# hydradarpa/kalman-hydra

Hardware: AMD Instinct MI355X
Metric: frames/sec (Brox flow + EKF update) at 1024^2 (higher is better)
Workload: dtype f32 (flow, renders) / f64 (EKF sums and state)

## Files before the change

kalman-hydra_amd/csrc/dense_kernels.h:

```cpp
#pragma once
#include <hip/hip_runtime.h>
#include "ekf_kernels.h"
#include "host_block.h"

#define DNB 32
#define TTT_PF 3

__device__ __forceinline__ double d_rsqrt(double d)
{
    const double r = __builtin_amdgcn_rsq(d);
    const double e = fma(-(d * r), r, 1.0);
#ifdef HM_RSQRT_ORDER2
    return fma(r * 0.5, e, r);
#else
    return fma(r, fma(e, 0.375, 0.5) * e, r);
#endif
}

__device__ __forceinline__ double d_readlane(double v, int lane)
{
    const int lo = __builtin_amdgcn_readlane(__double2loint(v), lane);
    const int hi = __builtin_amdgcn_readlane(__double2hiint(v), lane);
    return __hiloint2double(hi, lo);
}
// ... 438 lines not shown
    const int jj = 16 * (wv & 1) + (lane & 15);
#pragma unroll
    for (int e = 0; e < 4; e++) {
        const int ii = 16 * (wv >> 1) + (lane >> 4) + 4 * e;
        if (ii < ni && jj < nj) {
            W[(size_t)(i0 + ii) * n + j0 + jj] = acc[e];
            W[(size_t)(j0 + jj) * n + i0 + ii] = acc[e];
        }
    }
}

__global__ __launch_bounds__(256) void k_assemble(const double *__restrict__ invW0, const double *__restrict__ H,
                                                  const double *__restrict__ X0, const double *__restrict__ X,
                                                  const double *__restrict__ Hz, double *__restrict__ A, int n, int rhs_row,
                                                  double *__restrict__ Lt)
{
    __shared__ double s[4];
    const int row = blockIdx.x;
    if (row == (int)gridDim.x - 1) {
        __shared__ double W[DNB][DNB + 1];
        const int nd = min(DNB, n);
        for (int e = threadIdx.x; e < DNB * DNB; e += 256) {
            const int i = e / DNB, j = e % DNB;
            W[i][j] = (i < nd && j < nd) ? invW0[(size_t)i * n + j] + H[(size_t)i * n + j] : (i == j ? 1.0 : 0.0);
        }
        __syncthreads();
        if (threadIdx.x < 64) chol32_tinv_wave(W, Lt, threadIdx.x);
        return;
    }
    if (row >= n) {
        if (row != rhs_row)
            for (int j = threadIdx.x; j < n; j += 256) A[(size_t)row * n + j] = 0.0;
        return;
    }
    double acc = 0.0;
    for (int j = threadIdx.x; j < n; j += 256) {
        const double h = H[(size_t)row * n + j];
        A[(size_t)row * n + j] = invW0[(size_t)row * n + j] + h;
        acc += h * (X0[j] + -1.0 * X[j]);
    }
    for (int o = 32; o > 0; o >>= 1) acc += __shfl_down(acc, o, 64);
    if ((threadIdx.x & 63) == 0) s[threadIdx.x >> 6] = acc;
    __syncthreads();
    if (threadIdx.x == 0) A[(size_t)rhs_row * n + row] = Hz[row] - (((s[0] + s[1]) + s[2]) + s[3]);
}

#define RES_HEAD 10

__global__ __launch_bounds__(256) void k_iter_result(const double *__restrict__ step, int n, const double *__restrict__ partial,
                                                     int ntiles, const int *__restrict__ overflow,
                                                     const unsigned *__restrict__ flow_ctl, double *__restrict__ res, double ticket,
                                                     int delay_us)
{
    __shared__ double sp[RI_GROUPS * RI_NV];
    __shared__ double sums[RI_NV];
    const int t = threadIdx.x;
    const unsigned long long stamp = hb_stamp((long long)ticket);
    d_tile_partial_sums(partial, ntiles, sp, sums);
    __syncthreads();
    double v = 0.0;
    int slot = -1;
    if (t < 4) { slot = t; v = sums[t]; }
    else if (t == 4) { slot = 4; v = (double)*overflow; }
    else if (t == 5) { slot = 5; v = ticket; }
    else if (t == 6) { slot = 6; v = 0.0; }
    else if (t == 7) { slot = 7; v = (double)flow_ctl[1]; }
    else if (t == 8) { slot = 8; v = sums[4]; }
    else if (t == 9) { slot = 9; v = sums[5]; }
    if (delay_us > 0) {
        if (t == 9) { hb_put(res, n + 9, v, stamp); hb_flush(); }
        hb_delay(delay_us);
    }
    for (int i = t; i < n; i += 256) hb_put(res, i, step[i], stamp);
    if (slot >= 0) hb_put(res, n + slot, v, stamp);
    hb_flush();
}

__global__ __launch_bounds__(256) void k_gains(const double *__restrict__ W, const double *__restrict__ Hzc, int n,
                                               double *__restrict__ out)
{
    __shared__ double sm[3][4];
    const int row = blockIdx.x;
    double a0 = 0.0, a1 = 0.0, a2 = 0.0;
    for (int j = threadIdx.x; j < n; j += 256) {
        const double w = W[(size_t)row * n + j];
        const double *c = Hzc + (size_t)4 * j;
        a0 += w * c[0];
        a1 += w * (c[1] + c[2]);
        a2 += w * c[3];
    }
    for (int o = 32; o > 0; o >>= 1) {
        a0 += __shfl_down(a0, o, 64);
        a1 += __shfl_down(a1, o, 64);
        a2 += __shfl_down(a2, o, 64);
    }
    if ((threadIdx.x & 63) == 0) {
        sm[0][threadIdx.x >> 6] = a0;
        sm[1][threadIdx.x >> 6] = a1;
        sm[2][threadIdx.x >> 6] = a2;
    }
    __syncthreads();
    if (threadIdx.x < 3) {
        const double *q = sm[threadIdx.x];
        out[(size_t)threadIdx.x * n + row] = ((q[0] + q[1]) + q[2]) + q[3];
    }
}

__global__ __launch_bounds__(1024) void k_tail_result(const double *__restrict__ Hzc, const double *__restrict__ gain, int n,
                                                      double *__restrict__ blk, double ticket, int delay_us)
{
    const unsigned long long stamp = hb_stamp((long long)ticket);
    if (delay_us > 0) {
        if (threadIdx.x == 0) { hb_put(blk, 7 * n - 1, gain[3 * n - 1], stamp); hb_flush(); }
        hb_delay(delay_us);
    }
    for (int i = threadIdx.x; i < 4 * n; i += 1024) hb_put(blk, i, Hzc[i], stamp);
    for (int i = threadIdx.x; i < 3 * n; i += 1024) hb_put(blk, 4 * n + i, gain[i], stamp);
    hb_flush();
}

struct SpringTopo {
    const int *off;
    const int *bar;
    const int *other;
    const double *blk;
};

__global__ void k_fw_rows(const double *__restrict__ W, double *__restrict__ P, int N, SpringTopo tp, double a, double s)
// ... 47 lines not shown
```

kalman-hydra_amd/csrc/ekf.hip:

```cpp
#include "hm_common.h"
#include "ekf_kernels.h"
#include "dense_kernels.h"
#include "chol_flow_kernels.h"
#include "project_kernels.h"
#include "predict_kernels.h"
#include "view_kernels.h"
#include "body_kernels.h"
#include "smooth_kernels.h"
#include <algorithm>
#include <atomic>
#include <chrono>
#include <cmath>
#include <condition_variable>
#include <cstring>
#include <functional>
#include <mutex>
#include <set>
#include <thread>
#include <utility>
#include <vector>

struct Helper {
    std::thread th;
    std::mutex m;
// ... 52 lines not shown
    HmOwner own{1};
    Helper helper;
    bool helper_used = false;
    int tail_async = 1;
    double eps_Z, eps_J, eps_M;
    hipStream_t stream;
    int *d_tri, *d_star_off, *d_star_tri, *d_edges;
    int *d_nb_off = nullptr, *d_nb_u = nullptr, *d_nb_e = nullptr;
    float *d_uv;
    uint8_t *d_tex;
    std::vector<int> edges;
    uint8_t *d_yim, *d_ym;
    float *d_yfx, *d_yfy, *d_yfxm, *d_yfym;
    bool obs_owned = true;
    const uint8_t *o_yim, *o_ym;
    const float *o_yfx, *o_yfy;
    bool have_tex, have_obs, have_ref;
    Targets ref, P, Q;
    TriSetup *d_setup, *d_cfgs;
    int4 *d_ubox;
    int *d_tlist = nullptr, *d_tcount = nullptr;
    unsigned *d_tmask = nullptr;
    double *d_X, *d_out, *d_partial;
    uint8_t *d_im8, *d_m8;
    std::vector<double> X0;
    double *d_HTH;
    double *d_H, *d_Hz, *d_Hzc, *d_invW0, *d_Af[2], *d_T[2], *d_step, *d_Wtmp, *d_X0, *d_Xn, *d_Wprior, *d_gain, *d_Awork, *d_Lt[2];
    std::vector<double> upd_X0;
    int upd_last = -1, upd_prev = -1;
    double *d_Wres;
    double *pin;
    size_t pin_n;
    int *pin_scratch;
    std::vector<double> resv, tailv;
    int result_delay = 0;
    bool tail_pending = false;
    bool tail_valid = false;
    long long tail_ticket = 0;
    hipStream_t tail_stream = nullptr;
    const uint8_t *armed_mask = nullptr;
    std::vector<int> sp_h_off, sp_h_bar, sp_h_other;
    std::vector<double> sp_h_blk;
    std::vector<int32_t> sp_bars_cached;
    std::vector<int> tri;
    DPool pool;
    int *d_area;
    int *d_sp_off, *d_sp_bar, *d_sp_other;
    double *d_sp_blk;
    bool upd_open;
    bool prefactored;
    std::vector<double> h_partial;
    int red_blocks = 512;
    double *d_tpart = nullptr;
    std::vector<double> h_tpart;
    int ntiles = 0;
    int render_rows = RI_H;
    bool last_err_valid = false;
    double last_err[4] = {0, 0, 0, 0};
    std::vector<double> last_err_X;
    long long run_ticket;
    int vsplit = 5, esplit;
    bool pn_armed = false;
    void *pn_worker = nullptr;
    std::vector<int32_t> pn_bars;
    std::vector<double> pn_l0;
    double pn_par[4] = {0, 0, 0, 0};
    int pn_maxiter = 0;
    bool pq_armed = false;
    double pq_eps_F = 0.0;
    bool pq_valid = false;
    std::vector<double> pq_X, pq_l0;
    std::vector<int32_t> pq_bars;
    double pq_par[4] = {0, 0, 0, 0};
    hipStream_t stream3 = nullptr;
    int *d_n4nbr = nullptr, *d_n4nbb = nullptr, *d_n4bars = nullptr;
    double *d_n4l0 = nullptr;
    int n4deg = 0;
    std::vector<int32_t> n4_bars;
    std::vector<double> n4_l0;
    double *pin_n4 = nullptr;
    double *d_n4X = nullptr;
    std::vector<double> n4v;
    long long n4_ticket = 0;
    bool n4_pending = false;
    int newton_fail = 0;
    hipEvent_t ev_n4 = nullptr, ev_pm = nullptr;
    bool n4_ready = false;
    bool chain_pending = false;
    std::vector<double> chain_pred, chain_proj;
    int chain_its = 0, chain_moved = 0;
    double *pin_blk = nullptr;
    std::thread worker;
    bool worker_active;
    int worker_rc;
    char worker_err[512];
    int chol_flow = 1, flow_wgs = 192;
    int flow_stall = 0;
    int speculate = 1;
    double *d_flowP;
    unsigned *d_flowctl;
    hipStream_t stream2;
    hipStream_t stream4 = nullptr;
    hipEvent_t ev_tail = nullptr;
    bool tail_on_stream4 = false;
    int tail_split = 1;
    int *d_nbars, *d_nvoff, *d_nvbar, *d_ninfo;
// ... 243 lines not shown
            if (rc == HM_OK && 4 * ((int)nb[v].size() + 1) > PREP_MAX_ENTRIES) {
                hm_set_error("hm_ctx_create: vertex %d has %d neighbours, limit %d", v, (int)nb[v].size(), PREP_MAX_ENTRIES / 4 - 1);
                rc = HM_ERR_ARG;
            }
        }
        step(upload(h->own, &h->d_nb_off, noff.data(), noff.size()));
        step(upload(h->own, &h->d_nb_u, nu.data(), nu.size()));
        step(upload(h->own, &h->d_nb_e, ne.data(), ne.size()));
    }
    hipError_t e = hipSuccess;
    auto dev = [&](auto **p, size_t bytes) { if (e == hipSuccess) e = h->own.alloc(p, bytes); };
    if (rc == HM_OK) {
        const char *pe = getenv("HYDRA_MI_EKF_PRIORITY");
        e = h->own.stream(&h->stream, !(pe && atoi(pe) == 0));
        dev(&h->d_tex, n);
        dev(&h->d_yim, n);
        dev(&h->d_ym, n);
        dev(&h->d_yfx, n * sizeof(float));
        dev(&h->d_yfy, n * sizeof(float));
        dev(&h->d_yfxm, n * sizeof(float));
        dev(&h->d_yfym, n * sizeof(float));
        dev(&h->d_setup, (size_t)T * sizeof(TriSetup));
        dev(&h->d_cfgs, (size_t)N * MEAS_NCFG * (EKF_MAX_STAR + 1) * sizeof(TriSetup));
        dev(&h->d_ubox, (size_t)N * UBOX_STRIDE * sizeof(int4));
        dev(&h->d_tmask, (size_t)N * TMASK_STRIDE * sizeof(unsigned));
        dev(&h->d_tlist, (size_t)N * TMASK_STRIDE * sizeof(int));
        dev(&h->d_tcount, (size_t)N * sizeof(int));
        dev(&h->d_X, (size_t)4 * N * sizeof(double));
        dev(&h->d_out, (size_t)h->njobs * MEAS_VSPLIT_MAX * MEAS_OUT * sizeof(double));
        dev(&h->d_partial, (size_t)h->red_blocks * 4 * sizeof(double));
        h->ntiles = hm_cdiv(W, RI_W) * hm_cdiv(H, 8);
        dev(&h->d_tpart, (size_t)h->ntiles * RI_NV * sizeof(double));
        dev(&h->d_im8, n);
        dev(&h->d_m8, n);
        const size_t n4 = (size_t)4 * N, nn = n4 * n4 * sizeof(double);
        dev(&h->d_H, nn);
        dev(&h->d_HTH, nn);
        if (e == hipSuccess) e = hipMemsetAsync(h->d_HTH, 0, nn, h->stream);
        dev(&h->d_invW0, nn);
        const size_t nn_aug = (size_t)(hm_cdiv((int)n4, DNB) * DNB + DNB) * n4 * sizeof(double);
        dev(&h->d_Af[0], nn_aug);
        dev(&h->d_Af[1], nn_aug);
        dev(&h->d_Awork, nn_aug);
        const size_t ld_bytes = (size_t)hm_cdiv((int)n4, DNB) * DNB * DNB * sizeof(double);
        dev(&h->d_T[0], nn);
        dev(&h->d_T[1], nn);
        dev(&h->d_step, n4 * sizeof(double));
        dev(&h->d_Lt[0], ld_bytes);
        dev(&h->d_Lt[1], ld_bytes);
        dev(&h->d_Wtmp, nn);
        dev(&h->d_flowP, 3 * ld_bytes);
        dev(&h->d_flowctl, 4 * sizeof(unsigned));
        if (e == hipSuccess) e = hipMemsetAsync(h->d_flowctl, 0, 4 * sizeof(unsigned), h->stream);
        dev(&h->d_Hz, n4 * sizeof(double));
        dev(&h->d_Hzc, n4 * 4 * sizeof(double));
        dev(&h->d_Wprior, nn);
        dev(&h->d_gain, n4 * 3 * sizeof(double));
        h->pin_n = 2 * (n4 + RES_HEAD + n4 * 4 + n4 * 3) + 2;
        if (e == hipSuccess) e = h->own.host_alloc(&h->pin, h->pin_n * sizeof(double), hipHostMallocCoherent);
        if (e == hipSuccess) memset(h->pin, 0, h->pin_n * sizeof(double));
        h->pin_scratch = (int *)(h->pin + h->pin_n - 2);
        h->resv.assign(n4 + RES_HEAD, 0.0);
        h->tailv.assign(n4 * 7, 0.0);
        dev(&h->d_X0, n4 * sizeof(double));
        dev(&h->pool.hdr, (size_t)4 * N * sizeof(int));
        dev(&h->pool.overflow, sizeof(int));
        dev(&h->d_area, (size_t)N * sizeof(int));
        h->pool.area = h->d_area;
        if (e == hipSuccess) e = pool_alloc(h, (long long)8 * W * H);
        dev(&h->d_Xn, n4 * sizeof(double));
        for (Targets *t : {&h->ref, &h->P, &h->Q})
            if (e == hipSuccess) e = alloc_targets(h->own, *t, n);
    }
    if (e != hipSuccess) {
        hm_set_error("hm_ctx_create: device allocation failed: %s", hipGetErrorString(e));
        step(HM_ERR_HIP);
    }
    if (rc != HM_OK) {
        ctx_free(h);
        return rc;
    }
    h->h_partial.resize((size_t)h->red_blocks * 4);
    h->h_tpart.resize((size_t)h->ntiles * RI_NV);
    *out = h;
    return HM_OK;
}

extern "C" int hm_ctx_destroy(hm_ctx_t h) { return ctx_free(h); }

#ifdef HM_STAMP
extern "C" int hm_debug_stamps(void *dev_ptr)
{
    long long *p = (long long *)dev_ptr;
    HM_HIP(hipMemcpyToSymbol(HIP_SYMBOL(g_stamp), &p, sizeof p));
    return HM_OK;
}
#endif

extern "C" int hm_ctx_tune(hm_ctx_t h, const char *key, int value)
{
    HM_ARG(h != nullptr && key != nullptr, "hm_ctx_tune: NULL argument");
    HM_JOIN(h);
    if (!strcmp(key, "measure_split")) {
        HM_ARG(value >= 1 && value <= MEAS_VSPLIT_MAX, "hm_ctx_tune: measure_split must be in 1..%d", MEAS_VSPLIT_MAX);
        h->vsplit = value;
    } else if (!strcmp(key, "chol_flow")) {
        HM_ARG(value == 0 || value == 1, "hm_ctx_tune: chol_flow must be 0 (one launch per block step) or 1 (one persistent launch)");
        h->chol_flow = value;
    } else if (!strcmp(key, "chol_flow_wgs")) {
        HM_ARG(value >= 2 && value <= 2048, "hm_ctx_tune: chol_flow_wgs must be in 2..2048 (the chain workgroup and at least one task workgroup)");
        h->flow_wgs = value;
    } else if (!strcmp(key, "render_rows")) {
        HM_ARG(value == 8 || value == 16, "hm_ctx_tune: render_rows must be 8 or 16");
        h->render_rows = value;
    } else if (!strcmp(key, "chol_flow_stall")) {
        HM_ARG(value >= 0 && value <= 100000, "hm_ctx_tune: chol_flow_stall must be in 0..100000");
        h->flow_stall = value;
    } else if (!strcmp(key, "result_delay")) {
        HM_ARG(value >= 0 && value <= 5000, "hm_ctx_tune: result_delay must be in 0..5000 (microseconds)");
        h->result_delay = value;
    } else if (!strcmp(key, "tail_async")) {
        HM_ARG(value == 0 || value == 1, "hm_ctx_tune: tail_async must be 0 or 1");
        h->tail_async = value;
    } else if (!strcmp(key, "tail_split")) {
        HM_ARG(value == 0 || value == 1, "hm_ctx_tune: tail_split must be 0 or 1");
        h->tail_split = value;
    } else if (!strcmp(key, "newton_fail")) {
        HM_ARG(value == 0 || value == 1, "hm_ctx_tune: newton_fail must be 0 or 1");
        h->newton_fail = value;
    } else if (!strcmp(key, "speculate")) {
        HM_ARG(value == 0 || value == 1, "hm_ctx_tune: speculate must be 0 or 1");
        h->speculate = value;
    } else if (!strcmp(key, "edge_split")) {
        HM_ARG(value >= 1 && value <= MEAS_VSPLIT_MAX, "hm_ctx_tune: edge_split must be in 1..%d", MEAS_VSPLIT_MAX);
        h->esplit = value;
    } else {
        hm_set_error("hm_ctx_tune: unknown key '%s'", key);
        return HM_ERR_ARG;
    }
    return HM_OK;
}
extern "C" void *hm_ctx_stream(hm_ctx_t h)
{
    (void)ctx_join(h);
    return h ? (void *)h->stream : nullptr;
}
extern "C" int hm_ctx_sync(hm_ctx_t h)
{
    HM_ARG(h != nullptr, "hm_ctx_sync: NULL handle");
    HM_JOIN(h);
    HM_HIP(hipSetDevice(h->device));
    HM_HIP(hipStreamSynchronize(h->stream));
    return HM_OK;
}

extern "C" int hm_set_texture(hm_ctx_t h, const uint8_t *tex)
{
    HM_ARG(h && tex, "hm_set_texture: NULL argument");
    HM_JOIN(h);
    HM_HIP(hipSetDevice(h->device));
    HM_HIP(hipMemcpyAsync(h->d_tex, tex, (size_t)h->W * h->H, hipMemcpyHostToDevice, h->stream));
    HM_HIP(hipStreamSynchronize(h->stream));
    h->last_err_valid = false;
    h->have_tex = true;
    return HM_OK;
}

static int ensure_stream2(hm_ctx *h)
{
    HM_HIP(h->own.stream(&h->stream2));
    return HM_OK;
}

static int project_buffers(hm_ctx *h)
{
    if (h->pm_ready) return HM_OK;
    const size_t n = (size_t)h->W * h->H, n4 = (size_t)4 * h->N;
    HM_HIP(h->own.alloc(&h->d_outline, n * sizeof(int2)));
    HM_HIP(h->own.alloc(&h->d_outline_cnt, 4 * sizeof(int)));
    HM_HIP(h->own.alloc(&h->d_pm_flag, n));
    HM_HIP(h->own.alloc(&h->d_pm_pruned, n));
    HM_HIP(h->own.alloc(&h->ccl.L, n * sizeof(int)));
    HM_HIP(h->own.alloc(&h->ccl.cnt, n * sizeof(int)));
    HM_HIP(h->own.alloc(&h->ccl.bnd, n * sizeof(int)));
    HM_HIP(h->own.alloc(&h->ccl.edge, n));
// ... 55 lines not shown
    h->o_yim = h->d_yim; h->o_ym = h->d_ym; h->o_yfx = h->d_yfx; h->o_yfy = h->d_yfy;
    int rc = finish_observation(h);
    if (rc) return rc;
    HM_HIP(hipStreamSynchronize(h->stream));
    h->outline_ready = false;
    if (h->d_outline) {
        rc = queue_outline(h, h->o_ym);
        if (rc) return rc;
        h->outline_ready = true;
    }
    return HM_OK;
}

extern "C" int hm_set_observation_dev(hm_ctx_t h, const uint8_t *d_y_im, const float *d_y_fx, const float *d_y_fy,
                                      const uint8_t *d_y_m)
{
    HM_ARG(h && d_y_im && d_y_fx && d_y_fy && d_y_m, "hm_set_observation_dev: NULL argument");
    HM_JOIN_LAZY(h);
    HM_HIP(hipSetDevice(h->device));
    h->o_yim = d_y_im; h->o_ym = d_y_m; h->o_yfx = d_y_fx; h->o_yfy = d_y_fy;
    int rc = finish_observation(h);
    if (rc) return rc;
    h->outline_ready = false;
    if (h->d_outline && h->prepared_mask == d_y_m) {
        h->outline_ready = true;
    } else if (h->d_outline) {
        rc = queue_outline(h, h->o_ym);
        if (rc) return rc;
        h->outline_ready = true;
    }
    h->prepared_mask = nullptr;
    return HM_OK;
}

static int render_dev(hm_ctx *h, const double *dX, Targets t)
{
    Mesh m = {h->W, h->H, h->N, h->T, h->d_tri, h->d_uv, h->d_tex};
    hipLaunchKernelGGL(k_setup_all, dim3(hm_cdiv(h->T, 64)), dim3(64), 0, h->stream, m, dX, h->d_setup);
    hipLaunchKernelGGL((k_render<0>), dim3(hm_cdiv(h->W, EKF_TILE), hm_cdiv(h->H, EKF_TILE)), dim3(EKF_TILE, EKF_TILE), 0,
                       h->stream, m, dX, h->d_setup, t, (const int *)nullptr, (int *)nullptr);
    HM_HIP(hipGetLastError());
    return HM_OK;
}

static int render_into(hm_ctx *h, const double *X, Targets t)
{
    HM_HIP(hipMemcpyAsync(h->d_X, X, (size_t)4 * h->N * sizeof(double), hipMemcpyHostToDevice, h->stream));
    return render_dev(h, h->d_X, t);
}

static void measure_args(hm_ctx *h, const double *dX, double deltaX, int masked, MeasureArgs &a);
static int render_strips(const hm_ctx *h) { return hm_cdiv(h->W, RI_W) * hm_cdiv(h->H, h->render_rows); }

static int render_iter(hm_ctx *h, const double *dX, Targets t, bool with_err, int masked, bool regions, double deltaX)
{
    IterRenderArgs r;
    r.m = Mesh{h->W, h->H, h->N, h->T, h->d_tri, h->d_uv, h->d_tex};
    r.X = dX;
    r.out = t;
    r.o = Obs{h->o_yim, masked ? h->d_yfxm : h->o_yfx, masked ? h->d_yfym : h->o_yfy, h->o_ym};
    r.raw_fx = h->o_yfx; r.raw_fy = h->o_yfy;
    r.partial = h->d_tpart;
    r.tiles_x = hm_cdiv(h->W, RI_W); r.tiles_y = hm_cdiv(h->H, h->render_rows);
    const int nstrips = r.tiles_x * r.tiles_y;
    r.with_err = with_err ? 1 : 0;
    r.n_regions = regions ? h->N : 0;
    MeasureArgs a;
    measure_args(h, dX, deltaX, masked, a);
    if (h->render_rows == 8) hipLaunchKernelGGL((k_render_iter<8>), dim3(r.n_regions + nstrips), dim3(256), 0, h->stream, r, a, h->d_area);
    else hipLaunchKernelGGL((k_render_iter<16>), dim3(r.n_regions + nstrips), dim3(256), 0, h->stream, r, a, h->d_area);
    HM_HIP(hipGetLastError());
    return HM_OK;
}

static void hm_tile_partial_sums(const double *p, int ntiles, double s[RI_NV])
{
    static thread_local double g[RI_GROUPS][RI_NV];
    for (int t = 0; t < RI_GROUPS; t++) {
        double a[RI_NV];
        for (int k = 0; k < RI_NV; k++) a[k] = 0.0;
        for (int i = t; i < ntiles; i += RI_GROUPS)
            for (int k = 0; k < RI_NV; k++) a[k] += p[RI_NV * (size_t)i + k];
        for (int k = 0; k < RI_NV; k++) g[t][k] = a[k];
    }
    for (int k = 0; k < RI_NV; k++) {
        double v = 0.0;
        for (int t = 0; t < RI_GROUPS; t++) v += g[t][k];
        s[k] = v;
    }
}

#define NEED_TEX(h, who) \
    if (!(h)->have_tex) { hm_set_error(who ": hm_set_texture has not been called"); return HM_ERR_STATE; }
#define NEED_OBS(h, who) \
    if (!(h)->have_obs) { hm_set_error(who ": hm_set_observation has not been called"); return HM_ERR_STATE; }
#define NEED_REF(h, who) \
    if (!(h)->have_ref) { hm_set_error(who ": hm_initjacobian has not been called"); return HM_ERR_STATE; }

extern "C" int hm_render(hm_ctx_t h, const double *X, uint8_t *im, float *fx, float *fy, uint8_t *mk)
{
    HM_ARG(h && X, "hm_render: NULL argument");
    HM_JOIN(h);
    NEED_TEX(h, "hm_render");
    HM_HIP(hipSetDevice(h->device));
    int rc = render_into(h, X, h->P);
    if (rc) return rc;
    const int n = h->W * h->H;
    hipLaunchKernelGGL(k_resolve, dim3(hm_cdiv(n, 256)), dim3(256), 0, h->stream, h->P, h->d_im8, h->d_m8, n);
    if (im) HM_HIP(hipMemcpyAsync(im, h->d_im8, n, hipMemcpyDeviceToHost, h->stream));
    if (mk) HM_HIP(hipMemcpyAsync(mk, h->d_m8, n, hipMemcpyDeviceToHost, h->stream));
    if (fx) HM_HIP(hipMemcpyAsync(fx, h->P.fx, (size_t)n * sizeof(float), hipMemcpyDeviceToHost, h->stream));
    if (fy) HM_HIP(hipMemcpyAsync(fy, h->P.fy, (size_t)n * sizeof(float), hipMemcpyDeviceToHost, h->stream));
    HM_HIP(hipStreamSynchronize(h->stream));
    return HM_OK;
}

static Obs obs_of(hm_ctx *h, int masked)
{
    Obs o = {h->o_yim, masked ? h->d_yfxm : h->o_yfx, masked ? h->d_yfym : h->o_yfy, h->o_ym};
// ... 671 lines not shown
    const auto dbg_a = std::chrono::steady_clock::now();
    auto dbg_ms = [&]() { return std::chrono::duration<double, std::milli>(std::chrono::steady_clock::now() - dbg_a).count(); };
    double dbg_stage[8] = {0, 0, 0, 0, 0, 0, 0, 0};
    int rc = update_begin(h, W_prior, chained ? nullptr : X);
    if (rc) return rc;
    dbg_stage[0] = dbg_ms();
    const int N = h->N, n4 = 4 * N;
    std::vector<double> X0, Xcur, Xold;
    if (!chained) { X0.assign(X, X + n4); Xcur = X0; Xold = X0; }
    auto chain_collect = [&]() -> int {
        int r = hb_wait(h->stream3, h->pin_n4 + n4, 0, (size_t)n4 + 2, hb_stamp(h->n4_ticket), h->n4v.data(), "hm_update_run (state prediction)");
        h->n4_pending = false;
        if (r) return r;
        r = hb_wait(h->stream3, h->pin_pm + n4, 0, (size_t)n4 + 1, hb_stamp(h->pm_ticket), h->pmv.data(), "hm_update_run (projectmask)");
        if (r) return r;
        h->chain_pred.assign(h->n4v.begin(), h->n4v.begin() + n4);
        h->chain_proj.assign(h->pmv.begin(), h->pmv.begin() + n4);
        h->chain_its = (int)h->n4v[n4];
        h->chain_moved = (int)h->pmv[n4];
        if (h->n4v[n4 + 1] != 0.0) return 2;
        X0 = h->chain_proj; Xcur = X0; Xold = X0;
        h->upd_X0 = X0;
        h->X0 = X0;
        return HM_OK;
    };
    bool collected = !chained;
    if (!chained) HM_HIP(hipMemcpyAsync(h->d_X, h->d_X0, (size_t)n4 * sizeof(double), hipMemcpyDeviceToDevice, h->stream));
    double *const pin_res = h->pin, *const pin_tail = h->pin + 2 * ((size_t)n4 + RES_HEAD);
    const double *const res = h->resv.data();
    int niter = 0, accepted = 0;
    bool reverted = false, conv = false, ref_ready = false, regions_ahead = false, grown = false;
    double eold = 0.0;
    bool spec = false;
    auto unspec = [&]() {
        if (spec) { std::swap(h->ref, h->P); std::swap(h->d_X, h->d_Xn); spec = false; }
    };
    for (int it = 0; it < max_iter; it++) {
        if (!spec) {
            rc = measure_dev(h, h->d_X, ref_ready, deltaX, masked, regions_ahead, false);
            if (rc) return rc;
        }
        spec = false;
        if (next_mask && it == 0) {
            HM_HIP(h->own.event(&h->ev_m0));
            HM_HIP(hipEventRecord(h->ev_m0, h->stream));
        }
        if (collected) h->X0 = Xcur;
        h->have_ref = true;
        const int slot = h->upd_last == 0 ? 1 : 0;
        rc = ctx_join(h);
        if (rc) return rc;
        double *rhs_row = solve_step(h, slot, deltaX);
        regions_ahead = it + 1 < max_iter;
        rc = render_iter(h, h->d_Xn, h->P, true, masked, regions_ahead, deltaX);
        if (rc) return rc;
        hipLaunchKernelGGL(k_iter_result, dim3(1), dim3(256), 0, h->stream, rhs_row, n4, h->d_tpart,
                           render_strips(h), h->pool.overflow, (const unsigned *)h->d_flowctl, pin_res, (double)(++h->run_ticket),
                           h->result_delay);
        HM_HIP(hipGetLastError());
        if (h->speculate && regions_ahead) {
            std::swap(h->ref, h->P);
            std::swap(h->d_X, h->d_Xn);
            spec = true;
            rc = measure_dev(h, h->d_X, true, deltaX, masked, true, false);
            if (rc) { unspec(); return rc; }
        }
        const auto dbg_t0 = std::chrono::steady_clock::now();
        if (next_mask && it == 0) {
            rc = ensure_stream2(h);
            if (rc == HM_OK) { HM_HIP(hipStreamWaitEvent(h->stream2, h->ev_m0, 0)); rc = prepare_mask(h, next_mask); }
            if (rc) { unspec(); return rc; }
            next_mask = nullptr;
        }
        if (!collected) {
            rc = chain_collect();
            if (rc) { unspec(); (void)hipStreamSynchronize(h->stream); return rc; }
            collected = true;
        }
        rc = hb_wait(h->stream, pin_res, 0, (size_t)n4 + RES_HEAD, hb_stamp(h->run_ticket), h->resv.data(), "hm_update_run");
        if (rc) { unspec(); return rc; }
        if (getenv("HYDRA_MI_TRACE")) {
            const double ms = std::chrono::duration<double, std::milli>(std::chrono::steady_clock::now() - dbg_t0).count();
            if (ms > 1.5) fprintf(stderr, "[hydra_mi] hm_update_run: iteration %d waited %.2f ms for its result\n", it, ms);
        }
        if (res[n4 + 4] != 0.0) {
            unspec();
            if (grown) { hm_set_error("hm_update_run: the star regions do not fit the difference-image pool"); return HM_ERR_STATE; }
            if (regions_ahead) {
                MeasureArgs a;
                measure_args(h, h->d_X, deltaX, masked, a);
                hipLaunchKernelGGL(k_star_regions, dim3(h->N), dim3(REGION_NT), 0, h->stream, a, h->d_area);
                HM_HIP(hipGetLastError());
            }
            HM_HIP(hipStreamSynchronize(h->stream));
            rc = pool_grow(h, "hm_update_run");
            if (rc) return rc;
            grown = true;
            regions_ahead = false;
            HM_HIP(hipMemsetAsync(h->d_flowctl, 0, 4 * sizeof(unsigned), h->stream));
            it--;
            continue;
        }
        grown = false;
        h->upd_prev = h->upd_last;
        h->upd_last = slot;
        niter++;
        if (res[n4 + 7] != 0.0) {
            unspec();
            hm_set_error("hm_update_run: the factorisation launch gave up waiting for a block (chol_flow time-out)");
            return HM_ERR_HIP;
        }
        bool finite = true;
// ... 1114 lines not shown
```

kalman-hydra_amd/csrc/ekf_kernels.h:

```cpp
#pragma once
#include <hip/hip_runtime.h>
#include <stdint.h>

#define EKF_SUB 256
#define EKF_MAX_STAR 24
#define EKF_TILE 16
#define EKF_MAX_TRI 4096

struct TriSetup {
    double ea[3], eb[3], ec[3];
    double ecb[3];
    int cmin, cmax, rmin, rmax;
    int tl[3];
    float inv;
    int i0, i1, i2;
    float ux[3], uy[3], ax[3], ay[3];
};

__device__ __forceinline__ void d_tri_attr(TriSetup &s, const float *__restrict__ uv, const double *__restrict__ X, int N)
{
    const int id[3] = {s.i0, s.i1, s.i2};
    for (int k = 0; k < 3; k++) {
        s.ux[k] = uv[2 * id[k]];
        s.uy[k] = uv[2 * id[k] + 1];
        s.ax[k] = (float)X[2 * N + 2 * id[k]];
        s.ay[k] = (float)(-X[2 * N + 2 * id[k] + 1]);
    }
}

__device__ __forceinline__ long long d_snap(double x) { return (long long)rint(x * (double)EKF_SUB); }

__device__ __forceinline__ bool d_tri_sane(long long x0, long long y0, long long x1, long long y1, long long x2, long long y2)
{
    const long long lim = (long long)1 << 32;
    return x0 > -lim && x0 < lim && y0 > -lim && y0 < lim && x1 > -lim && x1 < lim && y1 > -lim && y1 < lim &&
           x2 > -lim && x2 < lim && y2 > -lim && y2 < lim;
}
__device__ __forceinline__ void d_tri_bbox(long long x0, long long y0, long long x1, long long y1, long long x2, long long y2,
                                           int W, int H, int &cmin, int &cmax, int &rmin, int &rmax)
{
    cmin = 1; cmax = 0; rmin = 1; rmax = 0;
    const long long area = d_tri_sane(x0, y0, x1, y1, x2, y2) ? (x1 - x0) * (y2 - y0) - (y1 - y0) * (x2 - x0) : 0;
    if (area == 0) return;
    long long xmin = x0 < x1 ? (x0 < x2 ? x0 : x2) : (x1 < x2 ? x1 : x2);
    long long xmax = x0 > x1 ? (x0 > x2 ? x0 : x2) : (x1 > x2 ? x1 : x2);
    long long ymin = y0 < y1 ? (y0 < y2 ? y0 : y2) : (y1 < y2 ? y1 : y2);
    long long ymax = y0 > y1 ? (y0 > y2 ? y0 : y2) : (y1 > y2 ? y1 : y2);
    long long cl = (xmin - 128) >> 8, ch = ((xmax - 128) >> 8) + 1;
    long long rl = (ymin - 128) >> 8, rh = ((ymax - 128) >> 8) + 1;
    if (cl < 0) cl = 0;
    if (rl < 0) rl = 0;
    if (ch > W - 1) ch = W - 1;
    if (rh > H - 1) rh = H - 1;
    cmin = (int)cl; cmax = (int)ch; rmin = (int)rl; rmax = (int)rh;
}
// ... 131 lines not shown
        if (s.cmin <= s.cmax && s.cmax >= c0 && s.cmin < c0 + EKF_TILE && s.rmax >= r0 && s.rmin < r0 + EKF_TILE)
            atomicOr(&s_mask[t >> 5], 1u << (t & 31));
    }
    __syncthreads();
    const int c = c0 + threadIdx.x, r = r0 + threadIdx.y;
    if (c >= m.W || r >= m.H) return;
    int acc = 0, cnt = 0, sg = 0, sb = 0;
    float fx = 0.0f, fy = 0.0f;
    for (int wd = 0; wd < words; wd++) {
        unsigned bits = s_mask[wd];
        while (bits) {
            int b = __ffs(bits) - 1;
            bits &= bits - 1;
            const TriSetup &s = setup[wd * 32 + b];
            float l1, l2;
            if (!d_tri_eval(s, c, r, l1, l2)) continue;
            if (MODE != 2) {
                acc += d_texel(m.tex, s, l1, l2, m.W, m.H);
                fx = fx + d_lerp(s.ax[0], s.ax[1], s.ax[2], l1, l2);
                fy = fy + d_lerp(s.ay[0], s.ay[1], s.ay[2], l1, l2);
                cnt++;
            }
            if (MODE != 0) {
                const int lab = labels[wd * 32 + b];
                sg += lab < 0 ? 255 : lab / 256;
                sb += lab < 0 ? 255 : lab % 256;
            }
        }
    }
    const int p = r * m.W + c;
    if (MODE != 2) { out.acc[p] = acc; out.fx[p] = fx; out.fy[p] = fy; out.cnt[p] = cnt; }
    if (MODE != 0) ids[p] = 256 * min(sg, 255) + min(sb, 255);
}

__global__ void k_resolve(Targets t, uint8_t *__restrict__ im, uint8_t *__restrict__ mk, int n)
{
    int p = blockIdx.x * blockDim.x + threadIdx.x;
    if (p >= n) return;
    if (im) im[p] = (uint8_t)(t.acc[p] > 255 ? 255 : t.acc[p]);
    if (mk) mk[p] = t.cnt[p] > 0 ? 255 : 0;
}

__global__ void k_mask_flow(const uint8_t *__restrict__ ym, const float *__restrict__ fx, const float *__restrict__ fy,
                            float *__restrict__ fxm, float *__restrict__ fym, int n)
{
    int p = blockIdx.x * blockDim.x + threadIdx.x;
    if (p >= n) return;
    float mm = (float)ym[p];
    fxm[p] = mm * fx[p];
    fym[p] = mm * fy[p];
}

template <int NACC, int NT>
__device__ inline void d_block_reduce(double (&a)[NACC], double *s_red , double *out)
{
#pragma unroll
    for (int k = 0; k < NACC; k++) {
        double v = a[k];
#pragma unroll
        for (int o = 32; o > 0; o >>= 1) v += __shfl_down(v, o, 64);
        a[k] = v;
    }
    const int lane = threadIdx.x & 63, wv = threadIdx.x >> 6;
    if (lane == 0)
        for (int k = 0; k < NACC; k++) s_red[wv * NACC + k] = a[k];
    __syncthreads();
    if (threadIdx.x < NACC) {
        double v = 0.0;
        for (int w = 0; w < NT / 64; w++) v += s_red[w * NACC + threadIdx.x];
        out[threadIdx.x] = v;
    }
}

struct Obs {
    const uint8_t *yim;
    const float *yfx, *yfy;
    const uint8_t *ym;
};

#define RED_NT 256
__global__ __launch_bounds__(RED_NT) void k_jz(Targets ref, Targets p, Obs o, int n, double *__restrict__ partial)
{
    __shared__ double s_red[(RED_NT / 64) * 4];
    double a[4] = {0, 0, 0, 0};
    for (int i = blockIdx.x * RED_NT + threadIdx.x; i < n; i += gridDim.x * RED_NT) {
        int rim = ref.acc[i] > 255 ? 255 : ref.acc[i], pim = p.acc[i] > 255 ? 255 : p.acc[i];
        int rm = ref.cnt[i] > 0 ? 255 : 0, pm = p.cnt[i] > 0 ? 255 : 0;
        double z = ((double)o.yim[i] - (double)rim) / 255.0;
        double zm = (255.0 * (double)o.ym[i] - (double)rm) / 255.0;
        float zfx = o.yfx[i] - ref.fx[i];
        float zfy = o.yfy[i] + ref.fy[i];
        a[0] += ((double)(pim - rim) / 255.0) * z;
        a[1] += (double)(p.fx[i] - ref.fx[i]) * (double)zfx;
        a[2] += (double)(p.fy[i] - ref.fy[i]) * (double)zfy;
        a[3] += ((double)(pm - rm) / 255.0) * zm;
    }
    d_block_reduce<4, RED_NT>(a, s_red, partial + 4 * blockIdx.x);
}

__global__ __launch_bounds__(RED_NT) void k_j(Targets ref, Targets p, Targets q, int n, double *__restrict__ partial)
{
    __shared__ double s_red[(RED_NT / 64) * 4];
    double a[4] = {0, 0, 0, 0};
    for (int i = blockIdx.x * RED_NT + threadIdx.x; i < n; i += gridDim.x * RED_NT) {
        int rim = ref.acc[i] > 255 ? 255 : ref.acc[i];
        int pim = p.acc[i] > 255 ? 255 : p.acc[i], qim = q.acc[i] > 255 ? 255 : q.acc[i];
        int rm = ref.cnt[i] > 0 ? 255 : 0, pm = p.cnt[i] > 0 ? 255 : 0, qm = q.cnt[i] > 0 ? 255 : 0;
        a[0] += ((double)(pim - rim) / 255.0) * ((double)(qim - rim) / 255.0);
        a[1] += (double)(p.fx[i] - ref.fx[i]) * (double)(q.fx[i] - ref.fx[i]);
        a[2] += (double)(p.fy[i] - ref.fy[i]) * (double)(q.fy[i] - ref.fy[i]);
        a[3] += ((double)(pm - rm) / 255.0) * ((double)(qm - rm) / 255.0);
    }
    d_block_reduce<4, RED_NT>(a, s_red, partial + 4 * blockIdx.x);
}

struct MultiArgs {
    Targets ref, p, q;
    const int *idr, *idp, *idq;
    Obs o;
    int W;
    const int4 *box;
    double *out;
};
// ... 554 lines not shown
        }
        unsigned long long todo = __ballot(go);
        if (todo == 0) continue;
        int l = __builtin_ctzll(todo);
        todo &= todo - 1;
        EdgeTile nx = d_edge_load(P, bv + (long long)__shfl(tv, l, 64) * 64 + lane, bw + (long long)__shfl(tw, l, 64) * 64 + lane);
        for (;;) {
            const EdgeTile t = nx;
            const bool more = todo != 0;
            if (more) {
                l = __builtin_ctzll(todo);
                todo &= todo - 1;
                nx = d_edge_load(P, bv + (long long)__shfl(tv, l, 64) * 64 + lane, bw + (long long)__shfl(tw, l, 64) * 64 + lane);
            }
            if (t.ax.x != POOL_EMPTY && t.bx.x != POOL_EMPTY) {
                const double axim = k255[t.ax.x], axm = k255[t.ax.y];
                const double ayim = k255[t.ay.x], aym = k255[t.ay.y];
                const double bxim = k255[t.bx.x], bxm = k255[t.bx.y];
                const double byim = k255[t.by.x], bym = k255[t.by.y];
                const double axfx = t.axfx, axfy = t.axfy, ayfx = t.ayfx, ayfy = t.ayfy;
                const double bxfx = t.bxfx, bxfy = t.bxfy, byfx = t.byfx, byfy = t.byfy;
                const double avx = t.avx, avy = t.avy, bvx = t.bvx, bvy = t.bvy;
                const double wxi = axim * iZ, wxf = axfx * iJ, wxg = axfy * iJ, wxm = axm * iM;
                const double wyi = ayim * iZ, wyf = ayfx * iJ, wyg = ayfy * iJ, wym = aym * iM;
                acc[B_XX] = fma(wxm, bxm, fma(wxg, bxfy, fma(wxf, bxfx, fma(wxi, bxim, acc[B_XX]))));
                acc[B_XY] = fma(wxm, bym, fma(wxg, byfy, fma(wxf, byfx, fma(wxi, byim, acc[B_XY]))));
                acc[B_YX] = fma(wym, bxm, fma(wyg, bxfy, fma(wyf, bxfx, fma(wyi, bxim, acc[B_YX]))));
                acc[B_YY] = fma(wym, bym, fma(wyg, byfy, fma(wyf, byfx, fma(wyi, byim, acc[B_YY]))));
                acc[B_XVX] = fma(axfx, bvx, acc[B_XVX]); acc[B_YVX] = fma(ayfx, bvx, acc[B_YVX]);
                acc[B_VXX] = fma(avx, bxfx, acc[B_VXX]); acc[B_VXY] = fma(avx, byfx, acc[B_VXY]);
                acc[B_VXVX] = fma(avx, bvx, acc[B_VXVX]);
                acc[B_XVY] = fma(axfy, bvy, acc[B_XVY]); acc[B_YVY] = fma(ayfy, bvy, acc[B_YVY]);
                acc[B_VYX] = fma(avy, bxfy, acc[B_VYX]); acc[B_VYY] = fma(avy, byfy, acc[B_VYY]);
                acc[B_VYVY] = fma(avy, bvy, acc[B_VYVY]);
            }
            if (!more) break;
        }
    }
    d_block_reduce<B_NV, MEAS_NT>(acc, s_red, a.out + ((size_t)(N + e) * MEAS_VSPLIT_MAX + blockIdx.y) * MEAS_OUT);
}

#define RI_CHUNK 32
#define RI_GROUPS 256
#define RI_W 64
#define RI_H 16
struct IterRenderArgs {
    Mesh m;
    const double *X;
    Targets out;
    Obs o;
    const float *raw_fx, *raw_fy;
    double *partial;
    int tiles_x, tiles_y, with_err, n_regions;
};
#define RI_NV 6
struct RenderShared {
    unsigned mask[EKF_MAX_TRI / 32];
    TriSetup cand[RI_CHUNK];
    double red[(256 / 64) * RI_NV];
    unsigned band[RI_W / 8];
};

#ifdef HM_STAMP
__device__ long long *g_stamp;
#define HM_STAMP_AT(k) do { if (g_stamp && threadIdx.x == 0) g_stamp[(size_t)blockIdx.x * 8 + (k)] = wall_clock64(); } while (0)
#else
#define HM_STAMP_AT(k) do { } while (0)
#endif
template <int RIH>
__global__ __launch_bounds__(256, 4) void k_render_iter(IterRenderArgs r, MeasureArgs a, int *__restrict__ area)
{
    HM_STAMP_AT(0);
    constexpr int RI_PX = RI_W * RIH / 256;
    __shared__ union {
        RegionShared reg;
        RenderShared t;
    } sh;
    if ((int)blockIdx.x < r.n_regions) {
        d_star_regions<256>(a, area, blockIdx.x, sh.reg);
        HM_STAMP_AT(4);
        return;
    }
    const Mesh &m = r.m;
    const int tile = blockIdx.x - r.n_regions;
    const int tid = threadIdx.x;
    const int words = (m.T + 31) / 32;
    for (int i = tid; i < words; i += 256) sh.t.mask[i] = 0;
    __syncthreads();
    const int c0 = (tile % r.tiles_x) * RI_W, r0 = (tile / r.tiles_x) * RIH;
    const double *__restrict__ X = r.X;
    for (int tb = tid; tb < m.T; tb += 512) {
        const int ta = tb, tc = tb + 256;
        const bool has2 = tc < m.T;
        const int a0 = m.tri[3 * ta], a1 = m.tri[3 * ta + 1], a2 = m.tri[3 * ta + 2];
        const int b0 = has2 ? m.tri[3 * tc] : a0, b1 = has2 ? m.tri[3 * tc + 1] : a1, b2 = has2 ? m.tri[3 * tc + 2] : a2;
        const double ax0 = X[2 * a0], ay0 = X[2 * a0 + 1], ax1 = X[2 * a1], ay1 = X[2 * a1 + 1], ax2 = X[2 * a2], ay2 = X[2 * a2 + 1];
        const double bx0 = X[2 * b0], by0 = X[2 * b0 + 1], bx1 = X[2 * b1], by1 = X[2 * b1 + 1], bx2 = X[2 * b2], by2 = X[2 * b2 + 1];
#pragma unroll
        for (int k = 0; k < 2; k++) {
            if (k == 1 && !has2) break;
            const int t = k ? tc : ta;
            const double x0 = k ? bx0 : ax0, y0 = k ? by0 : ay0, x1 = k ? bx1 : ax1, y1 = k ? by1 : ay1, x2 = k ? bx2 : ax2, y2 = k ? by2 : ay2;
            const double lo_x = fmin(x0, fmin(x1, x2)) - 2.0, hi_x = fmax(x0, fmax(x1, x2)) + 2.0;
            const double lo_y = fmin(y0, fmin(y1, y2)) - 2.0, hi_y = fmax(y0, fmax(y1, y2)) + 2.0;
            if (hi_x < (double)c0 || lo_x > (double)(c0 + RI_W) || hi_y < (double)r0 || lo_y > (double)(r0 + RIH)) continue;
            int cmin, cmax, rmin, rmax;
            d_tri_bbox(d_snap(x0), d_snap(y0), d_snap(x1), d_snap(y1), d_snap(x2), d_snap(y2), m.W, m.H, cmin, cmax, rmin, rmax);
            if (cmin <= cmax && cmax >= c0 && cmin < c0 + RI_W && rmax >= r0 && rmin < r0 + RIH)
                atomicOr(&sh.t.mask[t >> 5], 1u << (t & 31));
        }
    }
    __syncthreads();
    HM_STAMP_AT(1);
    int total = 0;
    for (int w = 0; w < words; w++) total += __popc(sh.t.mask[w]);
    const int c = c0 + (tid & 63), rb = r0 + (tid >> 6);
    int acc[RI_PX], cnt[RI_PX], tadr[RI_PX];
    float fx[RI_PX], fy[RI_PX];
#pragma unroll
    for (int q = 0; q < RI_PX; q++) { acc[q] = 0; cnt[q] = 0; fx[q] = 0.0f; fy[q] = 0.0f; tadr[q] = -1; }
    for (int base = 0; base < total; base += RI_CHUNK) {
        const int nch = min(RI_CHUNK, total - base);
        for (int tb = tid; tb < m.T; tb += 256) {
            const unsigned word = sh.t.mask[tb >> 5], bit = 1u << (tb & 31);
            if (!(word & bit)) continue;
            int rank = __popc(word & (bit - 1u));
            for (int w = 0; w < (tb >> 5); w++) rank += __popc(sh.t.mask[w]);
            if (rank < base || rank >= base + nch) continue;
            const int v0 = m.tri[3 * tb], v1 = m.tri[3 * tb + 1], v2 = m.tri[3 * tb + 2];
            TriSetup su;
// ... 37 lines not shown
        }
        __syncthreads();
        if (c < m.W)
            for (unsigned bm = sh.t.band[(tid & 63) >> 3]; bm != 0; bm &= bm - 1) {
                const TriSetup &su = sh.t.cand[__builtin_ctz(bm)];
#pragma unroll
                for (int j = 0; j < RI_PX; j++) {
                    float l1, l2;
                    if (!d_tri_eval(su, c, rb + 4 * j, l1, l2)) continue;
                    const int at = d_texel_at(su, l1, l2, m.W, m.H);
                    if (tadr[j] < 0) tadr[j] = at;
                    else acc[j] += m.tex[at];
                    fx[j] = fx[j] + d_lerp(su.ax[0], su.ax[1], su.ax[2], l1, l2);
                    fy[j] = fy[j] + d_lerp(su.ay[0], su.ay[1], su.ay[2], l1, l2);
                    cnt[j]++;
                }
            }
        __syncthreads();
    }
    HM_STAMP_AT(2);
    {
        int tx[RI_PX];
#pragma unroll
        for (int j = 0; j < RI_PX; j++) tx[j] = m.tex[tadr[j] < 0 ? 0 : tadr[j]];
#pragma unroll
        for (int j = 0; j < RI_PX; j++) acc[j] += tadr[j] < 0 ? 0 : tx[j];
    }
    double e[RI_NV] = {0.0, 0.0, 0.0, 0.0, 0.0, 0.0};
#pragma unroll
    for (int j = 0; j < RI_PX; j++) {
        const int rr = rb + 4 * j;
        if (c >= m.W || rr >= m.H) continue;
        const int p = rr * m.W + c;
        r.out.acc[p] = acc[j]; r.out.fx[p] = fx[j]; r.out.fy[p] = fy[j]; r.out.cnt[p] = cnt[j];
        if (r.with_err) {
            const unsigned rim = acc[j] > 255 ? 255 : acc[j];
            const unsigned rm = cnt[j] > 0 ? 255 : 0;
            const unsigned d = ((unsigned)r.o.yim[p] - rim) & 255u;
            const unsigned dm = ((255u * (unsigned)r.o.ym[p]) - rm) & 255u;
            const float dfx = r.o.yfx[p] - fx[j];
            const float dfy = r.o.yfy[p] + fy[j];
            e[0] += (double)((d * d) & 255u);
            e[1] += (double)dfx * (double)dfx;
            e[2] += (double)dfy * (double)dfy;
            e[3] += (double)((dm * dm) & 255u);
            const float gfx = r.raw_fx[p] - fx[j];
            const float gfy = r.raw_fy[p] + fy[j];
            e[4] += (double)gfx * (double)gfx;
            e[5] += (double)gfy * (double)gfy;
        }
    }
    HM_STAMP_AT(3);
    if (!r.with_err) return;
    d_block_reduce<RI_NV, 256>(e, sh.t.red, r.partial + RI_NV * (size_t)tile);
    HM_STAMP_AT(4);
}

__device__ __forceinline__ void d_tile_partial_sums(const double *__restrict__ partial, int ntiles, double *sp, double *out)
{
    const int t = threadIdx.x;
    if (t < RI_GROUPS) {
        double s[RI_NV];
#pragma unroll
        for (int k = 0; k < RI_NV; k++) s[k] = 0.0;
#pragma unroll 4
        for (int i = t; i < ntiles; i += RI_GROUPS) {
            const double2 *q = (const double2 *)(partial + RI_NV * (size_t)i);
#pragma unroll
            for (int k = 0; k < RI_NV / 2; k++) { const double2 v = q[k]; s[2 * k] += v.x; s[2 * k + 1] += v.y; }
        }
#pragma unroll
        for (int k = 0; k < RI_NV; k++) sp[RI_NV * t + k] = s[k];
    }
    __syncthreads();
    if (t < RI_NV) {
        double s = 0.0;
        for (int g = 0; g < RI_GROUPS; g++) s += sp[RI_NV * g + t];
        out[t] = s;
    }
}

struct ScatterArgs {
    const double *out;
    const int *edges;
    int N, E, vsplit, esplit;
    double eZ, eJ, eM, d;
    double *H, *Hz, *Hzc;
};

__device__ __forceinline__ void d_put(double *H, int n4, int p, int q, double val, double d)
{
    const double v = val / d / d;
    H[(size_t)p * n4 + q] = v;
    H[(size_t)q * n4 + p] = v;
}

__global__ __launch_bounds__(256) void k_hth_scatter(ScatterArgs a)
{
    __shared__ double so[4][MEAS_OUT];
    const int wv = threadIdx.x >> 6, lane = threadIdx.x & 63;
    const int job = blockIdx.x * 4 + wv;
    const int N = a.N, n4 = 4 * N;
    const bool on = job < N + a.E;
    if (on && lane < MEAS_OUT) {
        const double *src = a.out + (size_t)job * MEAS_VSPLIT_MAX * MEAS_OUT;
        const int parts = job < N ? a.vsplit : a.esplit;
        double v = src[lane];
        for (int q = 1; q < parts; q++) v += src[q * MEAS_OUT + lane];
        so[wv][lane] = v;
    }
    __syncthreads();
    if (!on) return;
    const double *o = so[wv];
    const double eZ = a.eZ, eJ = a.eJ, eM = a.eM, d = a.d;
    if (job < N) {
        const int v = job;
        const int idx[4] = {2 * v, 2 * v + 1, 2 * N + 2 * v, 2 * N + 2 * v + 1};
        if (lane < 4) {
            const int k = lane;
            double c[4] = {0.0, 0.0, 0.0, 0.0};
            if (k < 2) {
                const double *p = o + (k == 0 ? A_X : A_Y);
                c[0] = p[0] / eZ; c[1] = p[1] / eJ; c[2] = -p[2] / eJ; c[3] = p[3] / eM;
            } else if (k == 2) {
                c[1] = o[A_VX] / eJ;
            } else {
                c[2] = -o[A_VY] / eJ;
            }
            a.Hz[idx[k]] = (((c[0] + c[1]) + c[2]) + c[3]) / d / 2;
            for (int ch = 0; ch < 4; ch++) a.Hzc[(size_t)idx[k] * 4 + ch] = c[ch] / d / 2;
        } else if (lane >= 8 && lane < 17) {
            const int ix = idx[0], iy = idx[1], ivx = idx[2], ivy = idx[3];
// ... 36 lines not shown
```

Baseline: 334.6.

## Fold iteration result kernel into render kernel via last-block completion counter

Removes the separate single-block k_iter_result launch after each render_iter. Instead, each render tile writes its partial sums with agent-scope atomic stores and increments a device counter. The last block to finish reduces all partials and publishes the result to pinned host memory. This saves one kernel launch and its dependency gap per iteration, at the cost of an atomic per block and a serialized tail inside the render kernel.

```diff
diff --git a/kalman-hydra_amd/csrc/dense_kernels.h b/kalman-hydra_amd/csrc/dense_kernels.h
--- a/kalman-hydra_amd/csrc/dense_kernels.h
+++ b/kalman-hydra_amd/csrc/dense_kernels.h
@@ -514,28 +514,8 @@
                                                      const unsigned *__restrict__ flow_ctl, double *__restrict__ res, double ticket,
                                                      int delay_us)
 {
-    __shared__ double sp[RI_GROUPS * RI_NV];
-    __shared__ double sums[RI_NV];
-    const int t = threadIdx.x;
-    const unsigned long long stamp = hb_stamp((long long)ticket);
-    d_tile_partial_sums(partial, ntiles, sp, sums);
-    __syncthreads();
-    double v = 0.0;
-    int slot = -1;
-    if (t < 4) { slot = t; v = sums[t]; }
-    else if (t == 4) { slot = 4; v = (double)*overflow; }
-    else if (t == 5) { slot = 5; v = ticket; }
-    else if (t == 6) { slot = 6; v = 0.0; }
-    else if (t == 7) { slot = 7; v = (double)flow_ctl[1]; }
-    else if (t == 8) { slot = 8; v = sums[4]; }
-    else if (t == 9) { slot = 9; v = sums[5]; }
-    if (delay_us > 0) {
-        if (t == 9) { hb_put(res, n + 9, v, stamp); hb_flush(); }
-        hb_delay(delay_us);
-    }
-    for (int i = t; i < n; i += 256) hb_put(res, i, step[i], stamp);
-    if (slot >= 0) hb_put(res, n + slot, v, stamp);
-    hb_flush();
+    __shared__ ResultShared sh;
+    d_iter_result(step, n, partial, ntiles, overflow, flow_ctl, res, ticket, delay_us, sh);
 }
 
 __global__ __launch_bounds__(256) void k_gains(const double *__restrict__ W, const double *__restrict__ Hzc, int n,
diff --git a/kalman-hydra_amd/csrc/ekf.hip b/kalman-hydra_amd/csrc/ekf.hip
--- a/kalman-hydra_amd/csrc/ekf.hip
+++ b/kalman-hydra_amd/csrc/ekf.hip
@@ -128,6 +128,8 @@
     std::vector<double> h_partial;
     int red_blocks = 512;
     double *d_tpart = nullptr;
+    unsigned *d_ri_done = nullptr;
+    int iter_fold = 1;
     std::vector<double> h_tpart;
     int ntiles = 0;
     int render_rows = RI_H;
@@ -477,6 +479,8 @@
         dev(&h->d_flowP, 3 * ld_bytes);
         dev(&h->d_flowctl, 4 * sizeof(unsigned));
         if (e == hipSuccess) e = hipMemsetAsync(h->d_flowctl, 0, 4 * sizeof(unsigned), h->stream);
+        dev(&h->d_ri_done, sizeof(unsigned));
+        if (e == hipSuccess) e = hipMemsetAsync(h->d_ri_done, 0, sizeof(unsigned), h->stream);
         dev(&h->d_Hz, n4 * sizeof(double));
         dev(&h->d_Hzc, n4 * 4 * sizeof(double));
         dev(&h->d_Wprior, nn);
@@ -556,6 +560,9 @@
     } else if (!strcmp(key, "speculate")) {
         HM_ARG(value == 0 || value == 1, "hm_ctx_tune: speculate must be 0 or 1");
         h->speculate = value;
+    } else if (!strcmp(key, "iter_fold")) {
+        HM_ARG(value == 0 || value == 1, "hm_ctx_tune: iter_fold must be 0 or 1");
+        h->iter_fold = value;
     } else if (!strcmp(key, "edge_split")) {
         HM_ARG(value >= 1 && value <= MEAS_VSPLIT_MAX, "hm_ctx_tune: edge_split must be in 1..%d", MEAS_VSPLIT_MAX);
         h->esplit = value;
@@ -717,7 +724,8 @@
 static void measure_args(hm_ctx *h, const double *dX, double deltaX, int masked, MeasureArgs &a);
 static int render_strips(const hm_ctx *h) { return hm_cdiv(h->W, RI_W) * hm_cdiv(h->H, h->render_rows); }
 
-static int render_iter(hm_ctx *h, const double *dX, Targets t, bool with_err, int masked, bool regions, double deltaX)
+static int render_iter(hm_ctx *h, const double *dX, Targets t, bool with_err, int masked, bool regions, double deltaX,
+                       const double *step = nullptr, double *res = nullptr, double ticket = 0.0)
 {
     IterRenderArgs r;
     r.m = Mesh{h->W, h->H, h->N, h->T, h->d_tri, h->d_uv, h->d_tex};
@@ -730,6 +738,9 @@
     const int nstrips = r.tiles_x * r.tiles_y;
     r.with_err = with_err ? 1 : 0;
     r.n_regions = regions ? h->N : 0;
+    r.done = res ? h->d_ri_done : nullptr;
+    r.step = step; r.overflow = h->pool.overflow; r.flow_ctl = (const unsigned *)h->d_flowctl; r.res = res; r.ticket = ticket;
+    r.n = 4 * h->N; r.delay_us = h->result_delay;
     MeasureArgs a;
     measure_args(h, dX, deltaX, masked, a);
     if (h->render_rows == 8) hipLaunchKernelGGL((k_render_iter<8>), dim3(r.n_regions + nstrips), dim3(256), 0, h->stream, r, a, h->d_area);
@@ -1507,12 +1518,17 @@
         if (rc) return rc;
         double *rhs_row = solve_step(h, slot, deltaX);
         regions_ahead = it + 1 < max_iter;
-        rc = render_iter(h, h->d_Xn, h->P, true, masked, regions_ahead, deltaX);
-        if (rc) return rc;
-        hipLaunchKernelGGL(k_iter_result, dim3(1), dim3(256), 0, h->stream, rhs_row, n4, h->d_tpart,
-                           render_strips(h), h->pool.overflow, (const unsigned *)h->d_flowctl, pin_res, (double)(++h->run_ticket),
-                           h->result_delay);
-        HM_HIP(hipGetLastError());
+        if (h->iter_fold) {
+            rc = render_iter(h, h->d_Xn, h->P, true, masked, regions_ahead, deltaX, rhs_row, pin_res, (double)(++h->run_ticket));
+            if (rc) return rc;
+        } else {
+            rc = render_iter(h, h->d_Xn, h->P, true, masked, regions_ahead, deltaX);
+            if (rc) return rc;
+            hipLaunchKernelGGL(k_iter_result, dim3(1), dim3(256), 0, h->stream, rhs_row, n4, h->d_tpart,
+                               render_strips(h), h->pool.overflow, (const unsigned *)h->d_flowctl, pin_res, (double)(++h->run_ticket),
+                               h->result_delay);
+            HM_HIP(hipGetLastError());
+        }
         if (h->speculate && regions_ahead) {
             std::swap(h->ref, h->P);
             std::swap(h->d_X, h->d_Xn);
diff --git a/kalman-hydra_amd/csrc/ekf_kernels.h b/kalman-hydra_amd/csrc/ekf_kernels.h
--- a/kalman-hydra_amd/csrc/ekf_kernels.h
+++ b/kalman-hydra_amd/csrc/ekf_kernels.h
@@ -1,6 +1,7 @@
 #pragma once
 #include <hip/hip_runtime.h>
 #include <stdint.h>
+#include "host_block.h"
 
 #define EKF_SUB 256
 #define EKF_MAX_STAR 24
@@ -238,7 +239,7 @@
 }
 
 template <int NACC, int NT>
-__device__ inline void d_block_reduce(double (&a)[NACC], double *s_red , double *out)
+__device__ inline void d_block_reduce(double (&a)[NACC], double *s_red , double *out, bool coherent = false)
 {
 #pragma unroll
     for (int k = 0; k < NACC; k++) {
@@ -254,7 +255,11 @@
     if (threadIdx.x < NACC) {
         double v = 0.0;
         for (int w = 0; w < NT / 64; w++) v += s_red[w * NACC + threadIdx.x];
-        out[threadIdx.x] = v;
+        if (coherent)
+            __hip_atomic_store((unsigned long long *)out + threadIdx.x, (unsigned long long)__double_as_longlong(v),
+                               __ATOMIC_RELAXED, __HIP_MEMORY_SCOPE_AGENT);
+        else
+            out[threadIdx.x] = v;
     }
 }
 
@@ -915,6 +920,13 @@
     const float *raw_fx, *raw_fy;
     double *partial;
     int tiles_x, tiles_y, with_err, n_regions;
+    unsigned *done;
+    const double *step;
+    const int *overflow;
+    const unsigned *flow_ctl;
+    double *res;
+    double ticket;
+    int n, delay_us;
 };
 #define RI_NV 6
 struct RenderShared {
@@ -930,6 +942,17 @@
 #else
 #define HM_STAMP_AT(k) do { } while (0)
 #endif
+struct ResultShared {
+    double sp[RI_GROUPS * RI_NV];
+    double sums[RI_NV];
+};
+template <bool COHERENT = false>
+__device__ __forceinline__ void d_tile_partial_sums(const double *__restrict__ partial, int ntiles, double *sp, double *out);
+template <bool COHERENT = false>
+__device__ __forceinline__ void d_iter_result(const double *__restrict__ step, int n, const double *__restrict__ partial,
+                                              int ntiles, const int *__restrict__ overflow, const unsigned *__restrict__ flow_ctl,
+                                              double *__restrict__ res, double ticket, int delay_us, ResultShared &sh);
+
 template <int RIH>
 __global__ __launch_bounds__(256, 4) void k_render_iter(IterRenderArgs r, MeasureArgs a, int *__restrict__ area)
 {
@@ -938,7 +961,9 @@
     __shared__ union {
         RegionShared reg;
         RenderShared t;
+        ResultShared res;
     } sh;
+    __shared__ int s_last;
     if ((int)blockIdx.x < r.n_regions) {
         d_star_regions<256>(a, area, blockIdx.x, sh.reg);
         HM_STAMP_AT(4);
@@ -1082,10 +1107,21 @@
     }
     HM_STAMP_AT(3);
     if (!r.with_err) return;
-    d_block_reduce<RI_NV, 256>(e, sh.t.red, r.partial + RI_NV * (size_t)tile);
+    d_block_reduce<RI_NV, 256>(e, sh.t.red, r.partial + RI_NV * (size_t)tile, r.done != nullptr);
     HM_STAMP_AT(4);
-}
-
+    if (r.done == nullptr) return;
+    const int nstrips = r.tiles_x * r.tiles_y;
+    if (tid == 0) {
+        __builtin_amdgcn_s_waitcnt(0);
+        s_last = atomicAdd(r.done, 1u) == (unsigned)(nstrips - 1);
+    }
+    __syncthreads();
+    if (!s_last) return;
+    if (tid == 0) { __hip_atomic_store(r.done, 0u, __ATOMIC_RELAXED, __HIP_MEMORY_SCOPE_AGENT); __builtin_amdgcn_s_waitcnt(0); }
+    d_iter_result<true>(r.step, r.n, r.partial, nstrips, r.overflow, r.flow_ctl, r.res, r.ticket, r.delay_us, sh.res);
+}
+
+template <bool COHERENT>
 __device__ __forceinline__ void d_tile_partial_sums(const double *__restrict__ partial, int ntiles, double *sp, double *out)
 {
     const int t = threadIdx.x;
@@ -1095,9 +1131,19 @@
         for (int k = 0; k < RI_NV; k++) s[k] = 0.0;
 #pragma unroll 4
         for (int i = t; i < ntiles; i += RI_GROUPS) {
-            const double2 *q = (const double2 *)(partial + RI_NV * (size_t)i);
-#pragma unroll
-            for (int k = 0; k < RI_NV / 2; k++) { const double2 v = q[k]; s[2 * k] += v.x; s[2 * k + 1] += v.y; }
+            if (COHERENT) {
+                const unsigned long long *q = (const unsigned long long *)(partial + RI_NV * (size_t)i);
+                double v[RI_NV];
+#pragma unroll
+                for (int k = 0; k < RI_NV; k++)
+                    v[k] = __longlong_as_double((long long)__hip_atomic_load(q + k, __ATOMIC_RELAXED, __HIP_MEMORY_SCOPE_AGENT));
+#pragma unroll
+                for (int k = 0; k < RI_NV; k++) s[k] += v[k];
+            } else {
+                const double2 *q = (const double2 *)(partial + RI_NV * (size_t)i);
+#pragma unroll
+                for (int k = 0; k < RI_NV / 2; k++) { const double2 v = q[k]; s[2 * k] += v.x; s[2 * k + 1] += v.y; }
+            }
         }
 #pragma unroll
         for (int k = 0; k < RI_NV; k++) sp[RI_NV * t + k] = s[k];
@@ -1108,6 +1154,33 @@
         for (int g = 0; g < RI_GROUPS; g++) s += sp[RI_NV * g + t];
         out[t] = s;
     }
+}
+
+template <bool COHERENT>
+__device__ __forceinline__ void d_iter_result(const double *__restrict__ step, int n, const double *__restrict__ partial,
+                                              int ntiles, const int *__restrict__ overflow, const unsigned *__restrict__ flow_ctl,
+                                              double *__restrict__ res, double ticket, int delay_us, ResultShared &sh)
+{
+    const int t = threadIdx.x;
+    const unsigned long long stamp = hb_stamp((long long)ticket);
+    d_tile_partial_sums<COHERENT>(partial, ntiles, sh.sp, sh.sums);
+    __syncthreads();
+    double v = 0.0;
+    int slot = -1;
+    if (t < 4) { slot = t; v = sh.sums[t]; }
+    else if (t == 4) { slot = 4; v = (double)*overflow; }
+    else if (t == 5) { slot = 5; v = ticket; }
+    else if (t == 6) { slot = 6; v = 0.0; }
+    else if (t == 7) { slot = 7; v = (double)flow_ctl[1]; }
+    else if (t == 8) { slot = 8; v = sh.sums[4]; }
+    else if (t == 9) { slot = 9; v = sh.sums[5]; }
+    if (delay_us > 0) {
+        if (t == 9) { hb_put(res, n + 9, v, stamp); hb_flush(); }
+        hb_delay(delay_us);
+    }
+    for (int i = t; i < n; i += 256) hb_put(res, i, step[i], stamp);
+    if (slot >= 0) hb_put(res, n + slot, v, stamp);
+    hb_flush();
 }
 
 struct ScatterArgs {
```

Result: no change. 333.8 (median of 3 runs) (-0.2%).
